# ACMMM2021-Anonymous/video-graph-ssl

Hardware: AMD Instinct MI355X
Metric: pretrain_clips_per_sec (higher is better)
Workload: dtype bf16x6 (fp32 tensors; conv products as 6 bf16 MFMAs on hi/mid/lo splits = fp32-grade, fp32 accumulate; everything else fp32)

## Files before the change

include/gca_hip.h:

```cpp
#ifndef GCA_HIP_H
#define GCA_HIP_H

#include <stdint.h>

#ifdef __cplusplus
extern "C" {
#endif

#define GCA_OK 0
#define GCA_EINVAL (-1)
#define GCA_ELAUNCH (-2)

int gca_version(void);

int gca_conv_halo_occupancy(int tm, int tn, int math, int64_t lds_bytes);

int gca_set_conv_math(int mode);
int gca_get_conv_math(void);

typedef struct {
  int32_t N, C, D, H, W;
  int32_t K;
  int32_t kd, kh, kw;
  int32_t sd, sh, sw;
  int32_t pd, ph, pw;
  int32_t OD, OH, OW;
  int64_t x_batch_stride;
  int32_t tune_fwd_bm, tune_fwd_splits;
  int32_t tune_dgrad_bm, tune_dgrad_splits;
  int32_t tune_wgrad_splits, tune_wgrad_tile;
  int32_t tune_fwd_tail, tune_dgrad_tail;
  int32_t tune_fwd_math, tune_dgrad_math, tune_wgrad_math;
  int32_t tune_fwd_box, tune_dgrad_box;
  int32_t act_f16;
} gca_conv_geom;

int64_t gca_conv_pack_elems(const gca_conv_geom* g, int which);
int gca_conv_pack(const gca_conv_geom* g, int which, const float* w, float* packed, void* stream);

#define GCA_PACK_JOB_BYTES 128
int64_t gca_conv_pack_jobs_host(const gca_conv_geom* g, int which, const float* w, float* packed, void* jobs_out);
int64_t gca_conv_pack_jobs_finalize_host(void* jobs, int64_t njobs);
int gca_conv_pack_batched(const void* jobs_dev, int64_t njobs, int64_t total_blocks, void* stream);

int64_t gca_conv_table_rows(const gca_conv_geom* g, int which);
int gca_conv_table_build_host(const gca_conv_geom* g, int which, int32_t* table_host );

int64_t gca_conv_fwd_stat_parts(const gca_conv_geom* g);
int gca_conv_kernel_cfg(const gca_conv_geom* g, int which, int32_t* out4);
int64_t gca_conv_pack_layout(const gca_conv_geom* g, int which);
int64_t gca_conv_fwd_ws_bytes(const gca_conv_geom* g);
int gca_conv_fwd(const gca_conv_geom* g, const void* x, const float* wpack, const int32_t* table,
                 const float* bias, void* y, float* stat_sum, float* stat_sq, void* ws, void* stream);

int64_t gca_conv_dgrad_ws_bytes(const gca_conv_geom* g);
int gca_conv_dgrad(const gca_conv_geom* g, const void* dy, const float* wpack, const int32_t* table,
                   void* dx, int accumulate, void* ws, void* stream);

int64_t gca_conv_wgrad_ws_bytes(const gca_conv_geom* g);
int gca_conv_wgrad(const gca_conv_geom* g, const void* x, const void* dy, const int32_t* table,
                   float* dw, int accumulate, void* ws, void* stream);
typedef struct {
  const float* slabs;
  float* dw;
  int64_t n;
  int32_t splits, accumulate;
  int32_t first_block, nblocks;
} gca_reduce_job;
int gca_conv_wgrad_partial(const gca_conv_geom* g, const void* x, const float* in_scale, const float* in_shift, const void* dy,
                           const int32_t* table, void* slabs, int32_t* out_splits, void* stream);

int gca_conv_xf_ok(const gca_conv_geom* g);
int gca_conv_fwd_xf(const gca_conv_geom* g, const void* x, const float* in_scale, const float* in_shift, const float* wpack,
                    const int32_t* table, const float* bias, void* y, float* stat_sum, float* stat_sq, void* ws, void* stream);
int gca_conv_wgrad_xf(const gca_conv_geom* g, const void* x, const float* in_scale, const float* in_shift, const void* dy,
                      const int32_t* table, float* dw, int accumulate, void* ws, void* stream);
int gca_conv_dzf_ok(const gca_conv_geom* g);
int gca_conv_wgrad_dzf(const gca_conv_geom* g, const void* x, const void* dz, const void* y, const float* consts, int relu,
                       const int32_t* table, float* dw, int accumulate, void* ws, void* stream);
int gca_conv_wgrad_dzf_partial(const gca_conv_geom* g, const void* x, const void* dz, const void* y, const float* consts, int relu,
                               const int32_t* table, void* slabs, int32_t* out_splits, void* stream);
int64_t gca_reduce_jobs_finalize_host(gca_reduce_job* jobs, int64_t njobs);
int gca_splitk_reduce_batched(const gca_reduce_job* jobs_dev, int64_t njobs, int64_t total_blocks, void* stream);
int gca_conv_wgrad_cfg(const gca_conv_geom* g, int32_t* out4);

int gca_bias_grad(const float* dy, int64_t N, int64_t K, int64_t SP, float* db, int accumulate, void* stream);

int gca_bn_stats(const void* x, int64_t N, int64_t C, int64_t SP, float* stat_sum, float* stat_sq,
                 int64_t* parts_out, int act_f16, void* stream);
int64_t gca_bn_stats_parts(int64_t N, int64_t C, int64_t SP);
int gca_bn_finalize(const float* stat_sum, const float* stat_sq, int64_t P, int64_t C, double count,
                    const float* gamma, const float* beta, float eps, float momentum,
                    float* running_mean, float* running_var, int64_t* num_batches_tracked,
                    float* save_mean, float* save_invstd, float* scale, float* shift, void* stream);
int gca_conv_fwd_slabs(const gca_conv_geom* g, const void* x, const float* wpack, const int32_t* table, void* ws,
                       int32_t* out_splits, void* stream);
int gca_bn_train_fwd_slabs(const float* slabs, int64_t splits, double count, const float* gamma, const float* beta, float eps,
                           float momentum, float* running_mean, float* running_var, int64_t* num_batches_tracked,
                           float* save_mean, float* save_invstd, float* scale, float* shift, float* y, const float* residual,
                           int relu, int64_t N, int64_t C, int64_t SP, float* z, int64_t z_batch_stride, void* stream);
int gca_bn_train_fwd(const float* stat_sum, const float* stat_sq, int64_t P, int64_t C, double count,
                     const float* gamma, const float* beta, float eps, float momentum,
                     float* running_mean, float* running_var, int64_t* num_batches_tracked,
                     float* save_mean, float* save_invstd, float* scale, float* shift,
                     const void* x, const void* residual, int relu, int64_t N, int64_t SP, void* z,
                     int64_t z_batch_stride, int act_f16, void* stream);
int gca_bn_fold_eval(const float* gamma, const float* beta, const float* running_mean,
                     const float* running_var, float eps, int64_t C, float* scale, float* shift, void* stream);
int gca_bn_apply(const void* x, const float* scale, const float* shift, const void* residual,
                 int relu, int64_t N, int64_t C, int64_t SP, void* z, int64_t z_batch_stride, int act_f16, void* stream);
// ... 131 lines not shown
```

video-graph-ssl_amd/_hip.py:

```python
import ctypes as C
import os

import torch

_HERE = os.path.dirname(os.path.abspath(__file__))
LIB_PATH = os.environ.get('GCA_LIB_PATH') or os.path.join(_HERE, 'libgca_hip.so')


class HipLibraryMissing(RuntimeError):
    pass


if not os.path.exists(LIB_PATH):
    raise HipLibraryMissing(
        'libgca_hip.so is not built (%s). Run ./build_hip.sh or __graft_entry__.build(); there is no '
        'CPU fallback for the product path.' % LIB_PATH)
lib = C.CDLL(LIB_PATH)

c_i32, c_i64, c_f32, c_f64, c_vp = C.c_int32, C.c_int64, C.c_float, C.c_double, C.c_void_p


class ConvGeom(C.Structure):
    _fields_ = [(n, c_i32) for n in ('N', 'C', 'D', 'H', 'W', 'K', 'kd', 'kh', 'kw', 'sd', 'sh', 'sw',
                                     'pd', 'ph', 'pw', 'OD', 'OH', 'OW')] + [('x_batch_stride', c_i64)] + \
               [(n, c_i32) for n in ('tune_fwd_bm', 'tune_fwd_splits', 'tune_dgrad_bm', 'tune_dgrad_splits',
                                     'tune_wgrad_splits', 'tune_wgrad_tile', 'tune_fwd_tail', 'tune_dgrad_tail',
                                     'tune_fwd_math', 'tune_dgrad_math', 'tune_wgrad_math', 'tune_fwd_box',
                                     'tune_dgrad_box', 'act_f16')]


class PoolGeom(C.Structure):
    _fields_ = [(n, c_i32) for n in ('N', 'C', 'D', 'H', 'W', 'kd', 'kh', 'kw', 'sd', 'sh', 'sw',
                                     'pd', 'ph', 'pw', 'OD', 'OH', 'OW')]


_GP, _PP = C.POINTER(ConvGeom), C.POINTER(PoolGeom)
SIGNATURES = {
    'gca_version': (c_i32, []),
    'gca_conv_halo_occupancy': (c_i32, [c_i32, c_i32, c_i32, c_i64]),
    'gca_set_conv_math': (c_i32, [c_i32]),
    'gca_get_conv_math': (c_i32, []),
    'gca_conv_pack_elems': (c_i64, [_GP, c_i32]),
    'gca_conv_pack': (c_i32, [_GP, c_i32, c_vp, c_vp, c_vp]),
    'gca_conv_table_rows': (c_i64, [_GP, c_i32]),
    'gca_conv_table_build_host': (c_i32, [_GP, c_i32, c_vp]),
    'gca_conv_fwd_stat_parts': (c_i64, [_GP]),
    'gca_conv_kernel_cfg': (c_i32, [_GP, c_i32, c_vp]),
    'gca_conv_pack_layout': (c_i64, [_GP, c_i32]),
    'gca_conv_fwd_ws_bytes': (c_i64, [_GP]),
    'gca_conv_fwd': (c_i32, [_GP, c_vp, c_vp, c_vp, c_vp, c_vp, c_vp, c_vp, c_vp, c_vp]),
    'gca_conv_dgrad_ws_bytes': (c_i64, [_GP]),
    'gca_conv_dgrad': (c_i32, [_GP, c_vp, c_vp, c_vp, c_vp, c_i32, c_vp, c_vp]),
    'gca_conv_wgrad_cfg': (c_i32, [_GP, c_vp]),
    'gca_conv_wgrad_ws_bytes': (c_i64, [_GP]),
    'gca_conv_wgrad': (c_i32, [_GP, c_vp, c_vp, c_vp, c_vp, c_i32, c_vp, c_vp]),
    'gca_bias_grad': (c_i32, [c_vp, c_i64, c_i64, c_i64, c_vp, c_i32, c_vp]),
    'gca_bn_stats': (c_i32, [c_vp, c_i64, c_i64, c_i64, c_vp, c_vp, c_vp, c_i32, c_vp]),
    'gca_bn_stats_parts': (c_i64, [c_i64, c_i64, c_i64]),
    'gca_bn_finalize': (c_i32, [c_vp, c_vp, c_i64, c_i64, c_f64, c_vp, c_vp, c_f32, c_f32, c_vp, c_vp, c_vp,
                                c_vp, c_vp, c_vp, c_vp, c_vp]),
    'gca_bn_train_fwd': (c_i32, [c_vp, c_vp, c_i64, c_i64, c_f64, c_vp, c_vp, c_f32, c_f32, c_vp, c_vp, c_vp,
                                 c_vp, c_vp, c_vp, c_vp, c_vp, c_vp, c_i32, c_i64, c_i64, c_vp, c_i64, c_i32, c_vp]),
    'gca_bn_fold_eval': (c_i32, [c_vp, c_vp, c_vp, c_vp, c_f32, c_i64, c_vp, c_vp, c_vp]),
    'gca_bn_apply': (c_i32, [c_vp, c_vp, c_vp, c_vp, c_i32, c_i64, c_i64, c_i64, c_vp, c_i64, c_i32, c_vp]),
    'gca_bn_bwd_ws_bytes': (c_i64, [c_i64, c_i64, c_i64]),
    'gca_bn_bwd': (c_i32, [c_vp, c_vp, c_vp, c_vp, c_vp, c_vp, c_i32, c_i64, c_i64, c_i64, c_vp, c_vp, c_vp,
                           c_vp, c_i32, c_i64, c_vp, c_vp, c_vp, c_i32, c_vp]),
    'gca_maxpool3d_fwd': (c_i32, [_PP, c_vp, c_vp, c_vp, c_vp, c_vp, c_i32, c_vp]),
    'gca_maxpool3d_bwd': (c_i32, [_PP, c_vp, c_vp, c_vp, c_i32, c_i32, c_vp]),
    'gca_avgpool3d_fwd': (c_i32, [_PP, c_vp, c_vp, c_vp]),
    'gca_avgpool3d_bwd': (c_i32, [_PP, c_vp, c_vp, c_i32, c_vp]),
    'gca_wavgpool_fwd': (c_i32, [c_vp, c_vp, c_f32, c_i64, c_i64, c_i64, c_vp, c_i32, c_vp]),
    'gca_wavgpool_bwd': (c_i32, [c_vp, c_vp, c_f32, c_i64, c_i64, c_i64, c_vp, c_i32, c_vp]),
    'gca_relu_fwd': (c_i32, [c_vp, c_i64, c_vp, c_vp]),
    'gca_relu_bwd': (c_i32, [c_vp, c_vp, c_i64, c_vp, c_vp]),
    'gca_l2norm_fwd': (c_i32, [c_vp, c_i64, c_i64, c_f32, c_vp, c_vp, c_vp]),
    'gca_l2norm_bwd': (c_i32, [c_vp, c_vp, c_vp, c_i64, c_i64, c_vp, c_vp]),
    'gca_negcos_fwd_bwd': (c_i32, [c_vp, c_vp, c_i64, c_i64, c_f32, c_vp, c_i32, c_vp, c_vp]),
    'gca_infonce_ws_bytes': (c_i64, [c_i64, c_i64]),
    'gca_moco_logits_fwd': (c_i32, [c_vp, c_vp, c_vp, c_i64, c_i64, c_i64, c_f32, c_vp, c_vp, c_vp, c_vp, c_vp, c_vp, c_vp]),
    'gca_nce_softmax_loss_fwd': (c_i32, [c_vp, c_i64, c_i64, c_vp, c_vp, c_vp, c_vp]),
    'gca_nce_softmax_loss_bwd': (c_i32, [c_vp, c_vp, c_i64, c_i64, c_vp, c_f32, c_vp, c_vp]),
    'gca_moco_logits_bwd': (c_i32, [c_vp, c_vp, c_vp, c_vp, c_f32, c_vp, c_vp, c_i64, c_i64, c_i64, c_f32,
                                    c_i64, c_vp, c_i64, c_vp, c_vp, c_vp, c_vp]),
    'gca_queue_enqueue': (c_i32, [c_vp, c_i64, c_i64, c_vp, c_i64, c_i64, c_vp, c_vp, c_vp]),
    'gca_queue_advance': (c_i32, [c_vp, c_i64, c_i64, c_vp]),
    'gca_graph_gram_ws_bytes': (c_i64, [c_i64, c_i64, c_i64, c_i64]),
    'gca_graph_adj_fwd': (c_i32, [c_vp, c_vp, c_i64, c_i64, c_i64, c_i64, c_i32, c_f32, c_f32, c_vp, c_vp,
                                  c_vp, c_vp, c_vp, c_vp]),
    'gca_graph_adj_bwd': (c_i32, [c_vp, c_vp, c_vp, c_vp, c_vp, c_vp, c_i64, c_i64, c_i64, c_i64, c_i32, c_f32,
                                  c_f32, c_vp, c_vp, c_vp]),
    'gca_graph_gcn_fwd': (c_i32, [c_vp, c_vp, c_i64, c_i64, c_i64, c_i64, c_vp, c_vp]),
    'gca_graph_gcn_bwd_ws_bytes': (c_i64, [c_i64, c_i64, c_i64, c_i64]),
    'gca_graph_gcn_bwd': (c_i32, [c_vp, c_vp, c_vp, c_i64, c_i64, c_i64, c_i64, c_vp, c_vp, c_vp, c_vp]),
    'gca_ema_update': (c_i32, [c_vp, c_vp, c_i64, c_f32, c_vp]),
    'gca_sgd_step': (c_i32, [c_vp, c_vp, c_vp, c_i64, c_vp, c_vp, c_f32, c_f32, c_i32, c_i32, c_vp, c_vp]),
    'gca_lars_job_chunks': (c_i32, []),
    'gca_lars_step': (c_i32, [c_vp, c_vp, c_vp, c_i64, c_vp, c_vp, c_vp, c_i64, c_vp, c_vp, c_i64, c_vp, c_vp, c_vp, c_vp, c_f32,
                              c_i32, c_f64, c_f64, c_vp, c_vp]),
    'gca_adam_step': (c_i32, [c_vp, c_vp, c_vp, c_vp, c_i64, c_vp, c_vp, c_f64, c_f64, c_f64, c_i32, c_vp, c_vp, c_vp]),
    'gca_adam_advance': (c_i32, [c_vp, c_vp, c_vp]),
    'gca_grad_clip_ws_bytes': (c_i64, []),
    'gca_grad_clip_coef': (c_i32, [c_vp, c_i64, c_f32, c_vp, c_vp, c_vp]),
    'gca_conv_wgrad_partial': (c_i32, [_GP, c_vp, c_vp, c_vp, c_vp, c_vp, c_vp, c_vp, c_vp]),
    'gca_conv_xf_ok': (c_i32, [_GP]),
# ... 87 lines not shown
```

video-graph-ssl_amd/csrc/conv3d.hip:

```cpp
#include <cstring>
#include <type_traits>
#include "conv_halo.h"

#include <cstdlib>
#include <vector>

using namespace gca_conv;

namespace {


constexpr int LDK = BK + 4;
constexpr int lds_pitch(int math) { return math == 2 ? 28 : (math == 3 ? 12 : LDK); }
constexpr int lds_bufs(int tm, bool vec, int math) { return (math >= 1 || vec || tm >= 4) ? 1 : 2; }
constexpr int cmax(int a, int b) { return a > b ? a : b; }

template <int TM, int BN, int FAST, bool VEC, int MATH, bool H = false>
__device__ __forceinline__ void igemm_tile(
    const void* __restrict__ src, const float* __restrict__ apack, const int2* __restrict__ table,
    const float* __restrict__ bias, void* __restrict__ dst, float* __restrict__ psum,
    float* __restrict__ psq, float* __restrict__ slab, const IgemmParams p, int bid,
    float* __restrict__ As_, float* __restrict__ Bs_, int* __restrict__ taptab) {
  constexpr unsigned ES = H ? 2u : 4u;
  constexpr int BM = 32 * TM, TN = BN / 128;
// ... 537 lines not shown
      for (int r = 0; r < 16; ++r) {
        float s = 0.f, q = 0.f;
#pragma unroll
        for (int j = 0; j < TN; ++j) { const float v = acc[i][j][r]; s += v; q += v * v; }
        s = half_wave_sum_hi(s);
        q = half_wave_sum_hi(q);
        const int ro = i * 32 + (r & 3) + 8 * (r >> 2) + 4 * lh;
        if (ll == 31) { red[(wn * BM + ro) * 2] = s; red[(wn * BM + ro) * 2 + 1] = q; }
      }
    }
    __syncthreads();
    if (tid < BM && mbase + tid < p.DK) {
      const float s = red[tid * 2] + red[(BM + tid) * 2] + red[(2 * BM + tid) * 2] + red[(3 * BM + tid) * 2];
      const float q = red[tid * 2 + 1] + red[(BM + tid) * 2 + 1] + red[(2 * BM + tid) * 2 + 1] + red[(3 * BM + tid) * 2 + 1];
      const long long m = mbase + tid;
      psum[m * p.P + tileN] = s;
      psq[m * p.P + tileN] = q;
    }
  }
}

template <int TM, int BN, int FAST, bool VEC, int MATH, bool H = false>
__global__ __launch_bounds__(256) void conv_igemm_kernel(
    const void* __restrict__ src, const float* __restrict__ apack, const int2* __restrict__ table,
    const float* __restrict__ bias, void* __restrict__ dst, float* __restrict__ psum,
    float* __restrict__ psq, float* __restrict__ slab, IgemmParams p) {
  __shared__ __attribute__((aligned(16))) float As_[lds_bufs(TM, VEC, MATH) * 32 * TM * lds_pitch(MATH)];
  __shared__ __attribute__((aligned(16))) float Bs_[lds_bufs(TM, VEC, MATH) * BN * lds_pitch(MATH)];
  __shared__ int taptab[64];
  igemm_tile<TM, BN, FAST, VEC, MATH, H>(src, apack, table, bias, dst, psum, psq, slab, p, gca_xcd_remap(blockIdx.x, gridDim.x), As_, Bs_,
                                   taptab);
}

template <int TMA, int TMB, int FAST, int MATH>
__global__ __launch_bounds__(256) void conv_igemm_2phase_kernel(
    const void* __restrict__ src, const float* __restrict__ apack, const int2* __restrict__ table,
    const float* __restrict__ bias, void* __restrict__ dst, float* __restrict__ psum,
    float* __restrict__ psq, IgemmParams p, int nA, int tilesM_B, int tilesN_B) {
  static_assert(TMB < TMA, "the tail uses the shorter tile");
  __shared__ __attribute__((aligned(16))) float As_[cmax(lds_bufs(TMA, false, MATH) * TMA, lds_bufs(TMB, false, MATH) * TMB) * 32 * lds_pitch(MATH)];
  __shared__ __attribute__((aligned(16))) float Bs_[cmax(lds_bufs(TMA, false, MATH), lds_bufs(TMB, false, MATH)) * 128 * lds_pitch(MATH)];
  __shared__ int taptab[64];
  if ((int)blockIdx.x < nA) {
    igemm_tile<TMA, 128, FAST, false, MATH>(src, apack, table, bias, dst, psum, psq, nullptr, p, gca_xcd_remap(blockIdx.x, nA), As_, Bs_, taptab);
  } else {
    IgemmParams pb = p;
    pb.tileN_off = p.tileN_off + p.tilesN;
    pb.tilesM = tilesM_B; pb.tilesN = tilesN_B;
    igemm_tile<TMB, 128, FAST, false, MATH>(src, apack, table, bias, dst, psum, psq, nullptr, pb,
                                      gca_xcd_remap((int)blockIdx.x - nA, (int)gridDim.x - nA), As_, Bs_, taptab);
  }
}

constexpr int FINISH_CHUNK = 1024;
template <typename T>
__global__ __launch_bounds__(256) void conv_splitk_finish_kernel(
    const float* __restrict__ slab, int splits, const float* __restrict__ bias, T* __restrict__ dst,
    float* __restrict__ psum, float* __restrict__ psq, IgemmParams p) {
  __shared__ double sh[4];
  const int m = blockIdx.x, part = blockIdx.y, P = gridDim.y;
  const float b = bias ? bias[m] : 0.f;
  const long long lo = (long long)part * FINISH_CHUNK;
  long long hi = lo + FINISH_CHUNK; if (hi > p.Ntot) hi = p.Ntot;
  const int QSP = p.QD * p.QH * p.QW, QHW = p.QH * p.QW, DHW = p.DH * p.DW;
  const long long DSP = (long long)p.DD * DHW;
  double s = 0.0, q = 0.0;
  for (long long n = lo + threadIdx.x; n < hi; n += 256) {
    float v = 0.f;
    const float* sp0 = slab + (long long)m * p.Ntot + n;
    const long long sstride = (long long)p.DK * p.Ntot;
    int k = 0;
    for (; k + 4 <= splits; k += 4) {
      const float l0 = sp0[(long long)k * sstride], l1 = sp0[(long long)(k + 1) * sstride];
      const float l2 = sp0[(long long)(k + 2) * sstride], l3 = sp0[(long long)(k + 3) * sstride];
      v += l0; v += l1; v += l2; v += l3;
    }
    for (; k < splits; ++k) v += sp0[(long long)k * sstride];
    s += (double)v; q += (double)v * (double)v;
    v += b;
    const int img = (int)(n / QSP);
    const int sp = (int)(n - (long long)img * QSP);
    const int qd = sp / QHW, rr = sp - qd * QHW;
    const int qh = rr / p.QW, qw = rr - qh * p.QW;
    const long long dsp = (long long)(qd * p.dm_d + p.do_d) * DHW + (qh * p.dm_h + p.do_h) * p.DW + (qw * p.dm_w + p.do_w);
    T* d = dst + ((long long)img * p.DK + m) * DSP + dsp;
    if (p.accumulate) v += (float)*d;
    *d = (T)v;
  }
  if (psum) {
    s = gca_block_sum256_d(s, sh);
    q = gca_block_sum256_d(q, sh);
    if (threadIdx.x == 0) { psum[(long long)m * P + part] = (float)s; psq[(long long)m * P + part] = (float)q; }
  }
}

__device__ __forceinline__ void pack_elements(const float* __restrict__ w, float* __restrict__ packed,
                                              const PackParams& p, long long first, long long step, long long end) {
  for (long long i = first; i < end; i += step) {
    const int m = (int)(i / p.Kpad), k = (int)(i - (long long)m * p.Kpad);
    float v = 0.f;
    if (m < p.M && k < p.Kred) {
      const int ch = k / p.ntaps, tl = k - ch * p.ntaps;
      const int a = tl / (p.nb * p.nc), r = tl - a * (p.nb * p.nc), b = r / p.nc, c = r - b * p.nc;
      const int tap = ((p.k0d + p.sd * a) * p.KH + (p.k0h + p.sh * b)) * p.KW + (p.k0w + p.sw * c);
      v = w[(long long)ch * p.s_ch + tap + (long long)m * p.s_m];
    }
    packed[i] = v;
  }
}
__global__ void conv_pack_kernel(const float* __restrict__ w, float* __restrict__ packed, PackParams p) {
  if (p.fmt >= 1)
    pack_halo_elements(w, reinterpret_cast<unsigned char*>(packed), p, (long long)blockIdx.x * blockDim.x + threadIdx.x,
                       (long long)gridDim.x * blockDim.x, pack_items(p));
  else
    pack_elements(w, packed, p, (long long)blockIdx.x * blockDim.x + threadIdx.x, (long long)gridDim.x * blockDim.x,
                  pack_items(p));
}

constexpr int PACK_CHUNK = 2048;
struct PackJob {
  PackParams p;
  const float* w;
  float* packed;
  int first_block, nblocks;
};
static_assert(sizeof(PackJob) <= GCA_PACK_JOB_BYTES, "gca_hip.h: GCA_PACK_JOB_BYTES too small");
__global__ __launch_bounds__(256) void conv_pack_batched_kernel(const unsigned char* __restrict__ jobs, int njobs) {
  const int bid = blockIdx.x;
  int lo = 0, hi = njobs - 1;
  while (lo < hi) {
    const int mid = (lo + hi + 1) >> 1;
    if (reinterpret_cast<const PackJob*>(jobs + (size_t)mid * GCA_PACK_JOB_BYTES)->first_block <= bid) lo = mid;
    else hi = mid - 1;
  }
  const PackJob* j = reinterpret_cast<const PackJob*>(jobs + (size_t)lo * GCA_PACK_JOB_BYTES);
  const PackParams p = j->p;
  const long long base = (long long)(bid - j->first_block) * PACK_CHUNK;
  long long end = base + PACK_CHUNK;
  const long long total = pack_items(p);
  if (end > total) end = total;
  if (p.fmt >= 1) pack_halo_elements(j->w, reinterpret_cast<unsigned char*>(j->packed), p, base + threadIdx.x, 256, end);
  else pack_elements(j->w, j->packed, p, base + threadIdx.x, 256, end);
}

__global__ void zero_fill_kernel(unsigned* __restrict__ p, long long n32, int tail16) {
  for (long long i = (long long)blockIdx.x * blockDim.x + threadIdx.x; i < n32; i += (long long)gridDim.x * blockDim.x) p[i] = 0u;
// ... 387 lines not shown
  return pw_launch(pw, src, reinterpret_cast<const unsigned char*>(apack), bias, dst, psum, psq, st);
}

int run_class_stem(const gca_conv_geom* g, const IgemmCfg& cf, const float* src, const float* apack, const float* bias, float* dst,
                   float* psum, float* psq, const IgemmParams& p, hipStream_t st) {
  StemParams sp;
  if (!stem_geometry(g, p, cf.math, sp) || sp.bd != cf.bd || sp.bh != cf.bh || sp.bw != cf.bw) return GCA_EINVAL;
  sp.g.splits = 1; sp.g.kt_per_split = sp.nsteps;
  sp.g.tilesM = cdiv(p.DK, 32 * sp.wm);
  const long long tn = (long long)g->N * sp.nbd * sp.nbh * sp.nbw;
  if (tn > 0x7fffffffLL) return GCA_EINVAL;
  sp.g.tilesN = (int)tn; sp.g.tileN_off = 0;
  sp.g.P = (int)tn;
  return stem_launch(cf.math, sp, src, reinterpret_cast<const unsigned char*>(apack), bias, dst, psum, psq, st);
}

struct ConvLaunch {
  std::vector<ClassInfo> cls;
  std::vector<IgemmParams> p;
  std::vector<IgemmCfg> cf;
};

ConvLaunch resolve_launch(const gca_conv_geom* g, int which) {
  ConvLaunch L;
  build_classes(g, which, L.cls);
  const size_t n = L.cls.size();
  L.p.assign(n, IgemmParams{});
  L.cf.assign(n, IgemmCfg{});
  for (size_t i = 0; i < n; ++i) {
    if (L.cls[i].ntaps == 0) continue;
    class_params(g, which, L.cls[i], L.p[i]);
    L.cf[i] = cfg_for(g, which, L.cls[i], L.p[i], n);
  }
  return L;
}

int run_resolved_class(const gca_conv_geom* g, int which, const ConvLaunch& L, size_t i, const float* src, const float* apack,
                       const int2* table, const float* bias, float* dst, float* psum, float* psq, float* slab, int accumulate,
                       hipStream_t st, bool leave_slabs = false, const float* in_scale = nullptr, const float* in_shift = nullptr) {
  const ClassInfo& c = L.cls[i];
  const IgemmCfg& cf = L.cf[i];
  IgemmParams p = L.p[i];
  p.accumulate = accumulate ? 1 : 0;
  switch (cf.kernel) {
    case ConvKernel::Pointwise: return run_class_pw(g, which, src, apack, bias, dst, psum, psq, p, st);
    case ConvKernel::Stem: return run_class_stem(g, cf, src, apack, bias, dst, psum, psq, p, st);
    case ConvKernel::Halo:
      return run_class_halo(g, c, cf, src, apack, table, bias, dst, psum, psq, slab, p, st, leave_slabs, in_scale, in_shift);
    case ConvKernel::Gather: break;
  }
  return run_class(cf, fast_of(c.ntaps), src, apack, table, bias, dst, psum, psq, slab, p, st, leave_slabs);
}

int64_t ws_bytes_for(const gca_conv_geom* g, int which) {
  const ConvLaunch L = resolve_launch(g, which);
  int64_t need = 0;
  for (size_t i = 0; i < L.cls.size(); ++i)
    if (L.cf[i].splits > 1) need = std::max<int64_t>(need, (int64_t)L.cf[i].splits * L.p[i].DK * L.p[i].Ntot * (int64_t)sizeof(float));
  return need;
}

int g_conv_math = -1;

}

namespace gca_conv {
int conv_math() {
  if (g_conv_math < 0) {
    const char* e = getenv("GCA_CONV_MATH");
    g_conv_math = !e ? 2 : (!strcmp(e, "bf16x3") || !strcmp(e, "1")) ? 1 : (!strcmp(e, "f32") || !strcmp(e, "0")) ? 0 : 2;
  }
  return g_conv_math;
}
}

extern "C" {

int gca_version(void) { return 15; }

int gca_set_conv_math(int mode) {
  if (mode < 0 || mode > 2) return GCA_EINVAL;
  g_conv_math = mode;
  return GCA_OK;
}
int gca_get_conv_math(void) { return conv_math(); }

int64_t gca_conv_pack_elems(const gca_conv_geom* g, int which) {
  if (!geom_ok(g) || (which != 0 && which != 1)) return GCA_EINVAL;
  int64_t n = 0;
  for (const ClassInfo& c : resolve_launch(g, which).cls) n += pack_reserve(c);
  return n > 0 ? n : 64;
}

static void pack_params_of(const gca_conv_geom* g, int which, const ClassInfo& c, const IgemmCfg& cf, PackParams& p) {
  const int T = taps(g);
  p.fmt = (int)cf.kernel; p.math = cf.math; p.SC = c.srcC;
  p.nsteps = cf.kernel == ConvKernel::Stem ? cf.kt_per_split : cdiv(c.srcC, 16) * c.ntaps;
  const bool pwfmt = p.fmt == 3;
  p.Kred = (int)c.Kred; p.M = c.M; p.Kpad = pwfmt ? (int)gca_round_up(c.srcC, 32) : (int)c.Kpad; p.Mrows = pack_rows(c.M);
  p.ntaps = p.fmt == 2 ? g->kd * g->kh : c.ntaps; p.nb = c.nb; p.nc = c.nc;
  p.k0d = c.k0[0]; p.k0h = c.k0[1]; p.k0w = c.k0[2]; p.sd = c.ks[0]; p.sh = c.ks[1]; p.sw = c.ks[2];
  p.KH = g->kh; p.KW = g->kw; p.T = T;
  if (which == 0) { p.s_ch = T; p.s_m = (long long)g->C * T; }
  else { p.s_ch = (long long)g->C * T; p.s_m = T; }
}

int64_t gca_conv_pack_jobs_host(const gca_conv_geom* g, int which, const float* w, float* packed, void* jobs_out) {
  if (!geom_ok(g) || (which != 0 && which != 1)) return GCA_EINVAL;
  const ConvLaunch L = resolve_launch(g, which);
  int64_t n = 0;
  for (size_t i = 0; i < L.cls.size(); ++i) {
// ... 147 lines not shown
  if (!geom_ok(g)) return GCA_EINVAL;
  const ConvLaunch L = resolve_launch(g, 0);
  const IgemmCfg& cf = L.cf[0];
  if (cf.kernel == ConvKernel::Pointwise) return (int64_t)g->N * cdiv((int)((long long)g->OD * g->OH * g->OW), 128);
  return stat_parts(cf, L.p[0].Ntot, cf.kernel != ConvKernel::Gather ? halo_tiles_n(g, L.cls[0], cf) : 0);
}

int64_t gca_conv_fwd_ws_bytes(const gca_conv_geom* g) { return geom_ok(g) ? ws_bytes_for(g, 0) : GCA_EINVAL; }
int64_t gca_conv_dgrad_ws_bytes(const gca_conv_geom* g) { return geom_ok(g) ? ws_bytes_for(g, 1) : GCA_EINVAL; }

int gca_conv_fwd(const gca_conv_geom* g, const void* x_, const float* wpack, const int32_t* table,
                 const float* bias, void* y_, float* stat_sum, float* stat_sq, void* ws, void* stream) {
  const float* x = reinterpret_cast<const float*>(x_);
  float* y = reinterpret_cast<float*>(y_);
  if (!geom_ok(g) || !x || !wpack || !table || !y) return GCA_EINVAL;
  if ((stat_sum == nullptr) != (stat_sq == nullptr)) return GCA_EINVAL;
  return run_resolved_class(g, 0, resolve_launch(g, 0), 0, x, wpack, reinterpret_cast<const int2*>(table), bias, y, stat_sum,
                            stat_sq, reinterpret_cast<float*>(ws), 0, (hipStream_t)stream);
}

int gca_conv_fwd_slabs(const gca_conv_geom* g, const void* x, const float* wpack, const int32_t* table, void* ws,
                       int32_t* out_splits, void* stream) {
  if (!out_splits || !ws || !x || !wpack || !table || !geom_ok(g) || g->act_f16) return GCA_EINVAL;
  const ConvLaunch L = resolve_launch(g, 0);
  const IgemmCfg& cf = L.cf[0];
  if ((cf.kernel != ConvKernel::Gather && cf.kernel != ConvKernel::Halo) || cf.splits < 2) return GCA_EINVAL;
  float* slab = reinterpret_cast<float*>(ws);
  const int rc = run_resolved_class(g, 0, L, 0, reinterpret_cast<const float*>(x), wpack, reinterpret_cast<const int2*>(table),
                                    nullptr, slab, nullptr, nullptr, slab, 0, (hipStream_t)stream, true);
  if (rc) return rc;
  *out_splits = cf.splits;
  return GCA_OK;
}

int gca_conv_xf_ok(const gca_conv_geom* g) {
  if (!geom_ok(g) || g->act_f16) return 0;
  const IgemmCfg cf = resolve_launch(g, 0).cf[0];
  if (cf.kernel != ConvKernel::Halo || cf.math == 3) return 0;
  return resolve_wgrad(g).xf ? 1 : 0;
}

int gca_conv_fwd_xf(const gca_conv_geom* g, const void* x_, const float* in_scale, const float* in_shift, const float* wpack,
                    const int32_t* table, const float* bias, void* y_, float* stat_sum, float* stat_sq, void* ws, void* stream) {
  const float* x = reinterpret_cast<const float*>(x_);
  float* y = reinterpret_cast<float*>(y_);
  if (!geom_ok(g) || g->act_f16 || !x || !in_scale || !in_shift || !wpack || !table || !y) return GCA_EINVAL;
  if ((stat_sum == nullptr) != (stat_sq == nullptr)) return GCA_EINVAL;
  const ConvLaunch L = resolve_launch(g, 0);
  if (L.cf[0].kernel != ConvKernel::Halo) return GCA_EINVAL;
  return run_resolved_class(g, 0, L, 0, x, wpack, reinterpret_cast<const int2*>(table), bias, y, stat_sum, stat_sq,
                            reinterpret_cast<float*>(ws), 0, (hipStream_t)stream, false, in_scale, in_shift);
}

int gca_conv_dgrad(const gca_conv_geom* g, const void* dy_, const float* wpack, const int32_t* table,
                   void* dx_, int accumulate, void* ws, void* stream) {
  const float* dy = reinterpret_cast<const float*>(dy_);
  float* dx = reinterpret_cast<float*>(dx_);
  if (!geom_ok(g) || !dy || !wpack || !table || !dx) return GCA_EINVAL;
  if (g->x_batch_stride != 0 && g->x_batch_stride != (long long)g->C * g->D * g->H * g->W) return GCA_EINVAL;
  hipStream_t st = (hipStream_t)stream;
  const ConvLaunch L = resolve_launch(g, 1);
  bool any_empty = false;
  for (const ClassInfo& c : L.cls) any_empty |= c.ntaps == 0;
  if (any_empty && !accumulate) {
    const long long n = (long long)g->N * g->C * g->D * g->H * g->W;
    const long long n32 = g->act_f16 ? n / 2 : n;
    long long blocks = gca_ceil_div(n32 + 1, 1024);
    if (blocks > 4096) blocks = 4096;
    hipLaunchKernelGGL(zero_fill_kernel, dim3((unsigned)blocks), dim3(256), 0, st, reinterpret_cast<unsigned*>(dx), n32,
                       g->act_f16 ? (int)(n & 1) : 0);
  }
  const int2* tab = reinterpret_cast<const int2*>(table);
  for (size_t i = 0; i < L.cls.size(); ++i) {
    const ClassInfo& c = L.cls[i];
    if (c.ntaps == 0) continue;
    const int rc = run_resolved_class(g, 1, L, i, dy, wpack + c.pack_off, tab + c.table_off, nullptr, dx, nullptr, nullptr,
                                      reinterpret_cast<float*>(ws), accumulate, st);
    if (rc) return rc;
  }
  return GCA_OK;
}

}
```

video-graph-ssl_amd/csrc/conv_igemm_host.h:

```cpp
#pragma once
#include <algorithm>
#include <vector>
#include "conv_common.h"

namespace gca_conv {

struct IgemmParams {
  int SC, SD, SH, SW;
  int DK;
  int QD, QH, QW;
  int DD, DH, DW;
  int dm_d, dm_h, dm_w;
  int do_d, do_h, do_w;
  int m_d, m_h, m_w;
  int o_d, o_h, o_w;
  int ntaps;
  int Kpad, Mpad;
  int tilesM, tilesN;
  int tileN_off;
  int splits, kt_per_split;
  int P;
  int chk;
  int accumulate;
  long long Ntot;
  long long src_nstride;
  unsigned src_bytes;
  unsigned dst_bytes;
  unsigned slab_bytes;
};

struct ClassInfo {
  int na, nb, nc, ntaps;
  int k0[3], ks[3];
  int dl0[3], dls[3];
  int q[3];
  int dm[3], dof[3];
  int m[3], o[3];
  int srcC, M;
  long long Kred, Kpad;
  long long table_off;
  long long pack_off;
  bool vec;
};

inline int cdiv(int a, int b) { return (a + b - 1) / b; }
inline int fast_of(int ntaps) { return ntaps <= 31 ? 1 : (ntaps <= FAST_MAX_TAPS ? 2 : 0); }
inline int pack_rows(int M) { return (int)gca_round_up(M, 32) + 128; }

inline long long pack_reserve(const ClassInfo& c) {
  const long long rows = pack_rows(c.M);
  const long long flat = c.Kpad * rows;
  const long long halo = c.srcC >= 8 && c.ntaps <= 64 ? (long long)cdiv(c.srcC, 16) * c.ntaps * rows * 24 : 0;
  const long long stem = c.srcC <= 4 && c.nc <= 8 && c.m[2] == 2 ? (long long)cdiv(c.srcC * c.na * c.nb, 2) * rows * 24 : 0;
  const long long m = halo > stem ? halo : stem;
  return m > flat ? m : flat;
}

inline void build_classes(const gca_conv_geom* g, int which, std::vector<ClassInfo>& out) {
  const int kdim[3] = {g->kd, g->kh, g->kw}, sdim[3] = {g->sd, g->sh, g->sw}, pdim[3] = {g->pd, g->ph, g->pw};
  const int in[3] = {g->D, g->H, g->W}, od[3] = {g->OD, g->OH, g->OW};
  long long toff = 0, poff = 0;
  auto finish = [&](ClassInfo& c) {
    c.ntaps = c.na * c.nb * c.nc;
    c.Kred = (long long)c.srcC * c.ntaps;
    c.Kpad = gca_round_up(c.Kred, BK);
    c.table_off = toff; c.pack_off = poff;
    toff += c.Kpad + 32;
    poff += pack_reserve(c);
    const int SH = which == 0 ? in[1] : od[1], SW = which == 0 ? in[2] : od[2];
    c.vec = c.nb == 1 && c.nc == 1 && c.m[1] == 1 && c.m[2] == 1 && c.o[1] + c.dl0[1] == 0 && c.o[2] + c.dl0[2] == 0 &&
            c.dm[1] == 1 && c.dm[2] == 1 && c.dof[1] == 0 && c.dof[2] == 0 && c.q[1] == SH && c.q[2] == SW &&
            (SH * SW) % 4 == 0 && c.ntaps <= 31 &&
            (which == 1 || g->x_batch_stride % 4 == 0);
    out.push_back(c);
  };
  if (which == 0) {
    ClassInfo c{};
    c.na = g->kd; c.nb = g->kh; c.nc = g->kw;
    for (int d = 0; d < 3; ++d) {
      c.k0[d] = 0; c.ks[d] = 1; c.dl0[d] = 0; c.dls[d] = 1;
      c.q[d] = od[d]; c.dm[d] = 1; c.dof[d] = 0; c.m[d] = sdim[d]; c.o[d] = -pdim[d];
    }
// ... 84 lines not shown
```

video-graph-ssl_amd/engine/ops.py:

```python
import ctypes as C
import functools
import os

import torch

from .. import _hip as H
from .._hip import aptr, is_half, ptr, stream
from . import tune
from .tune import TUNE_HALO, TUNE_PW, TUNE_STEM, TUNE_VEC

F32 = torch.float32
F16 = torch.float16


def _t3(v):
    return (v, v, v) if isinstance(v, int) else tuple(int(a) for a in v)


class _Workspace:

    def __init__(self):
        self.buf = {}
        self.captured = set()
        self.retired = []
# ... 66 lines not shown

if _TUNE_PATH:
    import atexit
    if os.path.exists(_TUNE_PATH):
        load_tune_cache(_TUNE_PATH)
    atexit.register(lambda: _TUNE_DIRTY[0] and os.environ.get('RANK', '0') == '0' and save_tune_cache(_TUNE_PATH))


def _time_ms(fn, reps=3):
    fn()
    a, b = torch.cuda.Event(enable_timing=True), torch.cuda.Event(enable_timing=True)
    a.record()
    for _ in range(reps):
        fn()
    b.record()
    b.synchronize()
    return a.elapsed_time(b) / reps


_KERNELS = (('halo', TUNE_HALO, 14), ('stem', TUNE_STEM, 16), ('pw', TUNE_PW, 17))


def _tune_kernel(code):
    return next((name for name, flag, _ in _KERNELS if code & flag), 'gather')


class ConvPlan:

    def __init__(self, N, Cin, D, Hh, W, K, k, s, p, device, x_batch_stride=0, act_f16=False):
        kd, kh, kw = _t3(k)
        sd, sh, sw = _t3(s)
        pd, ph, pw = _t3(p)
        OD, OH, OW = (D + 2 * pd - kd) // sd + 1, (Hh + 2 * ph - kh) // sh + 1, (W + 2 * pw - kw) // sw + 1
        self.g = H.ConvGeom(N, Cin, D, Hh, W, K, kd, kh, kw, sd, sh, sw, pd, ph, pw, OD, OH, OW, x_batch_stride)
        self.g.act_f16 = int(bool(act_f16))
        self.act_dtype = F16 if act_f16 else F32
        self.gp = C.byref(self.g)
        self.in_shape = (N, Cin, D, Hh, W)
        self.out_shape = (N, K, OD, OH, OW)
        self.device = device
        self.taps = kd * kh * kw
        self._tables = {}
        self.tuned = [not AUTOTUNE] * 3
        if H.lib.gca_conv_fwd_stat_parts(self.gp) < 0:
            raise ValueError('unsupported conv geometry %r' % ((N, Cin, D, Hh, W, K, k, s, p),))
        self.pack_elems = [H.lib.gca_conv_pack_elems(self.gp, 0), H.lib.gca_conv_pack_elems(self.gp, 1)]
        self.refresh()

    def refresh(self):
        self.parts = H.lib.gca_conv_fwd_stat_parts(self.gp)
        self.wgrad_ws = H.lib.gca_conv_wgrad_ws_bytes(self.gp)
        self.fwd_ws = H.lib.gca_conv_fwd_ws_bytes(self.gp)
        self.dgrad_ws = H.lib.gca_conv_dgrad_ws_bytes(self.gp) if self.g.x_batch_stride == 0 else 0

    def table(self, which):
        t = self._tables.get(which)
        if t is None:
            rows = H.lib.gca_conv_table_rows(self.gp, which)
            host = torch.empty(rows * 2, dtype=torch.int32)
            H.call('gca_conv_table_build_host', self.gp, which, host.data_ptr())
            t = host.to(self.device)
            self._tables[which] = t
        return t

    def cfg(self, which):
        out = (C.c_int32 * 4)()
        if which == 2:
            H.call('gca_conv_wgrad_cfg', self.gp, out)
        else:
            H.call('gca_conv_kernel_cfg', self.gp, which, out)
        return tuple(out)

    WGRAD_KERNELS = {11: 'temporal32', 12: 'temporal64', 13: 'spatial', 14: 'stem'}
    WGRAD_SHAPES = tune.WGRAD_SHAPES

    def kernel(self, which):
        kc = self.cfg(which)[3]
        if which == 2:
            return self.WGRAD_KERNELS.get(kc & 255, 'gather')
        return next((name for name, _, bit in _KERNELS if kc >> bit & 1), 'gather')

    def math(self, which):
        return self.cfg(which)[3] >> 12 & 3

    def pack_layout(self, which):
        return 0 if which == 2 else H.lib.gca_conv_pack_layout(self.gp, which)

    def tune_key(self, which):
        g = self.g
        geom = (g.N, g.C, g.D, g.H, g.W, g.K, g.kd, g.kh, g.kw, g.sd, g.sh, g.sw, g.pd, g.ph, g.pw, g.x_batch_stride)
        return 'v%d%s:%d:%s' % (H.lib.gca_version(), 'h' if g.act_f16 else ('', 'b', 'c')[H.lib.gca_get_conv_math()], which,
                                ','.join(str(int(v)) for v in geom))

    def set_code(self, which, code):
        for field, v in zip(code._fields, code):
            setattr(self.g, 'tune_%s_%s' % (tune.PASSES[which], field), v)
        self.refresh()

    def tune(self, which, run, repack=None):
        if self.tuned[which] or torch.cuda.is_current_stream_capturing():
            return

        def measure():
            try:
                return _time_ms(run)
            except RuntimeError:
# ... 63 lines not shown

def conv_pack(plan, which, w, out=None):
    n = plan.pack_elems[which]
    if out is None or out.numel() != n:
        out = torch.zeros(n, dtype=F32, device=w.device)
    H.call('gca_conv_pack', plan.gp, which, ptr(w), ptr(out), stream())
    return out


def _act(plan, t):
    if t.dtype is not plan.act_dtype:
        raise TypeError('conv plan built for %s activations, got %s' % (plan.act_dtype, t.dtype))
    return aptr(t)


def _conv_fwd_launch(plan, x, wpack, bias, y, ss, sq):
    ws = WS.get(plan.fwd_ws, x.device) if plan.fwd_ws else None
    H.call('gca_conv_fwd', plan.gp, _act(plan, x), ptr(wpack), ptr(plan.table(0)), ptr(bias), _act(plan, y), ptr(ss), ptr(sq),
           ptr(ws), stream())


def _repacker(plan, which, w_raw, wpack):
    if w_raw is None:
        return None
    return lambda: H.call('gca_conv_pack', plan.gp, which, ptr(w_raw), ptr(wpack), stream())


def _stat_pair(plan, device):
    return tuple(torch.empty((plan.g.K, plan.parts), dtype=F32, device=device) for _ in range(2))


def conv_fwd(plan, x, wpack, bias=None, stats=False, w_raw=None):
    y = torch.empty(plan.out_shape, dtype=plan.act_dtype, device=x.device)
    if not plan.tuned[0]:
        plan.tune(0, lambda: _conv_fwd_launch(plan, x, wpack, bias, y, None, None), _repacker(plan, 0, w_raw, wpack))
    ss, sq = _stat_pair(plan, x.device) if stats else (None, None)
    _conv_fwd_launch(plan, x, wpack, bias, y, ss, sq)
    return (y, (ss, sq)) if stats else y


def conv_xf_ok(plan):
    return plan.tuned[0] and plan.tuned[2] and plan.g.x_batch_stride == 0 and bool(H.lib.gca_conv_xf_ok(plan.gp))


def conv_fwd_xf(plan, y_in, scale, shift, wpack, stats=False):
    y = torch.empty(plan.out_shape, dtype=F32, device=y_in.device)
    ss, sq = _stat_pair(plan, y_in.device) if stats else (None, None)
    ws = WS.get(plan.fwd_ws, y_in.device) if plan.fwd_ws else None
    H.call('gca_conv_fwd_xf', plan.gp, ptr(y_in), ptr(scale), ptr(shift), ptr(wpack), ptr(plan.table(0)), None, ptr(y), ptr(ss),
           ptr(sq), ptr(ws), stream())
    return (y, (ss, sq)) if stats else y


def _conv_dgrad_launch(plan, dy, wpack_t, dx, accumulate):
    ws = WS.get(plan.dgrad_ws, dy.device) if plan.dgrad_ws else None
    H.call('gca_conv_dgrad', plan.gp, _act(plan, dy), ptr(wpack_t), ptr(plan.table(1)), _act(plan, dx), int(accumulate), ptr(ws),
           stream())


def conv_dgrad(plan, dy, wpack_t, dx=None, accumulate=False, w_raw=None):
    if dx is None:
        dx = torch.empty(plan.in_shape, dtype=plan.act_dtype, device=dy.device)
        accumulate = False
    if not plan.tuned[1]:
        scratch = torch.empty(plan.in_shape, dtype=plan.act_dtype, device=dy.device)
        plan.tune(1, lambda: _conv_dgrad_launch(plan, dy, wpack_t, scratch, False), _repacker(plan, 1, w_raw, wpack_t))
    _conv_dgrad_launch(plan, dy, wpack_t, dx, accumulate)
    return dx


def _conv_wgrad_launch(plan, x, dy, dw, accumulate):
    ws = WS.get(plan.wgrad_ws, x.device)
    H.call('gca_conv_wgrad', plan.gp, _act(plan, x), _act(plan, dy), ptr(plan.table(2)), ptr(dw), int(accumulate), ptr(ws), stream())


class DeferredReduce(object):

    def __init__(self):
        self.slabs = {}
        self.tables = {}
        self.pending = []
        self.launches = 0

    def slab_for(self, dw, plan):
        key = (dw.data_ptr(), id(plan))
        b = self.slabs.get(key)
        if b is None or b.numel() < plan.wgrad_ws:
            if torch.cuda.is_current_stream_capturing():
                raise RuntimeError('weight-gradient slab would be allocated during graph capture; run one eager step first')
            b = self.slabs[key] = torch.empty(max(int(plan.wgrad_ws), 16), dtype=torch.uint8, device=dw.device)
        return b

    def add(self, plan, x, dy, dw, accumulate, xf=None, dzf=None):
        if any(j[1].data_ptr() == dw.data_ptr() for j in self.pending):
            self.flush()
        slab = self.slab_for(dw, plan)
        splits = C.c_int32(0)
        if dzf is not None:
            H.call('gca_conv_wgrad_dzf_partial', plan.gp, _act(plan, x), _act(plan, dy), _act(plan, dzf[0]), ptr(dzf[1]),
                   int(dzf[2]), ptr(plan.table(2)), slab.data_ptr(), C.addressof(splits), stream())
        else:
            H.call('gca_conv_wgrad_partial', plan.gp, _act(plan, x), ptr(xf[0]) if xf else None, ptr(xf[1]) if xf else None,
                   _act(plan, dy), ptr(plan.table(2)), slab.data_ptr(), C.addressof(splits), stream())
        self.pending.append((slab, dw, dw.numel(), int(splits.value), int(bool(accumulate))))

    def flush(self):
        if not self.pending:
            return
        jobs, self.pending = self.pending, []
        sig = tuple((j[0].data_ptr(), j[1].data_ptr(), j[2], j[3], j[4]) for j in jobs)
# ... 607 lines not shown
```

Before: 1656.

## Merge per-class strided dgrad launches into one multi-class kernel launch

Strided-conv dgrad used to issue a separate implicit-GEMM launch (plus a split-K finish launch) for each tap class. Now, when all classes share a tile config, one grouped kernel covers them, picking each workgroup's class from a prefix table passed as a kernel argument, and one finish kernel covers all split-K parts. This cuts launch count and lets classes fill the GPU together. In exchange the workspace grows to the sum of all class slabs instead of the max, and each block does a small class lookup.

```diff
diff --git a/include/gca_hip.h b/include/gca_hip.h
--- a/include/gca_hip.h
+++ b/include/gca_hip.h
@@ -56,6 +56,13 @@
 int64_t gca_conv_dgrad_ws_bytes(const gca_conv_geom* g);
 int gca_conv_dgrad(const gca_conv_geom* g, const void* dy, const float* wpack, const int32_t* table,
                    void* dx, int accumulate, void* ws, void* stream);
+#define GCA_CLASS_BLOCK_BYTES 2048
+int gca_conv_dgrad_merged(const gca_conv_geom* g, int64_t ws_bytes);
+int64_t gca_conv_dgrad_ws_bytes_merged(const gca_conv_geom* g);
+int gca_conv_dgrad_ws(const gca_conv_geom* g, const void* dy, const float* wpack, const int32_t* table,
+                      void* dx, int accumulate, void* ws, int64_t ws_bytes, void* stream);
+int gca_set_dgrad_merge(int on);
+int64_t gca_conv_class_block_bytes(void);
 
 int64_t gca_conv_wgrad_ws_bytes(const gca_conv_geom* g);
 int gca_conv_wgrad(const gca_conv_geom* g, const void* x, const void* dy, const int32_t* table,
diff --git a/video-graph-ssl_amd/_hip.py b/video-graph-ssl_amd/_hip.py
--- a/video-graph-ssl_amd/_hip.py
+++ b/video-graph-ssl_amd/_hip.py
@@ -51,6 +51,11 @@
     'gca_conv_fwd': (c_i32, [_GP, c_vp, c_vp, c_vp, c_vp, c_vp, c_vp, c_vp, c_vp, c_vp]),
     'gca_conv_dgrad_ws_bytes': (c_i64, [_GP]),
     'gca_conv_dgrad': (c_i32, [_GP, c_vp, c_vp, c_vp, c_vp, c_i32, c_vp, c_vp]),
+    'gca_conv_dgrad_ws_bytes_merged': (c_i64, [_GP]),
+    'gca_conv_dgrad_ws': (c_i32, [_GP, c_vp, c_vp, c_vp, c_vp, c_i32, c_vp, c_i64, c_vp]),
+    'gca_conv_dgrad_merged': (c_i32, [_GP, c_i64]),
+    'gca_set_dgrad_merge': (c_i32, [c_i32]),
+    'gca_conv_class_block_bytes': (c_i64, []),
     'gca_conv_wgrad_cfg': (c_i32, [_GP, c_vp]),
     'gca_conv_wgrad_ws_bytes': (c_i64, [_GP]),
     'gca_conv_wgrad': (c_i32, [_GP, c_vp, c_vp, c_vp, c_vp, c_i32, c_vp, c_vp]),
diff --git a/video-graph-ssl_amd/csrc/conv3d.hip b/video-graph-ssl_amd/csrc/conv3d.hip
--- a/video-graph-ssl_amd/csrc/conv3d.hip
+++ b/video-graph-ssl_amd/csrc/conv3d.hip
@@ -613,13 +613,32 @@
   }
 }
 
+__device__ __forceinline__ int class_of(const int* __restrict__ first, int id) {
+  int ci = 0;
+#pragma unroll
+  for (int i = 1; i < MAX_MERGED_CLASSES; ++i) ci += id >= first[i] ? 1 : 0;
+  return ci;
+}
+
+template <int TM, int BN, int FAST, bool VEC, int MATH, bool H = false>
+__global__ __launch_bounds__(256) void conv_igemm_classes_kernel(
+    const void* __restrict__ src, const float* __restrict__ apack, const int2* __restrict__ table, void* __restrict__ dst,
+    float* __restrict__ slab, const ClassBlock cb) {
+  __shared__ __attribute__((aligned(16))) float As_[lds_bufs(TM, VEC, MATH) * 32 * TM * lds_pitch(MATH)];
+  __shared__ __attribute__((aligned(16))) float Bs_[lds_bufs(TM, VEC, MATH) * BN * lds_pitch(MATH)];
+  __shared__ int taptab[64];
+  const int ci = class_of(cb.first_wg, (int)blockIdx.x);
+  const int first = cb.first_wg[ci], count = cb.first_wg[ci + 1] - first;
+  igemm_tile<TM, BN, FAST, VEC, MATH, H>(src, apack + cb.pack_off[ci], table + cb.table_off[ci], nullptr, dst, nullptr, nullptr,
+                                         slab + cb.slab_off[ci], cb.p[ci], gca_xcd_remap((int)blockIdx.x - first, count), As_, Bs_,
+                                         taptab);
+}
+
 constexpr int FINISH_CHUNK = 1024;
 template <typename T>
-__global__ __launch_bounds__(256) void conv_splitk_finish_kernel(
+__device__ __forceinline__ void splitk_finish_part(
     const float* __restrict__ slab, int splits, const float* __restrict__ bias, T* __restrict__ dst,
-    float* __restrict__ psum, float* __restrict__ psq, IgemmParams p) {
-  __shared__ double sh[4];
-  const int m = blockIdx.x, part = blockIdx.y, P = gridDim.y;
+    float* __restrict__ psum, float* __restrict__ psq, const IgemmParams& p, int m, int part, int P, double* sh) {
   const float b = bias ? bias[m] : 0.f;
   const long long lo = (long long)part * FINISH_CHUNK;
   long long hi = lo + FINISH_CHUNK; if (hi > p.Ntot) hi = p.Ntot;
@@ -653,6 +672,24 @@
     q = gca_block_sum256_d(q, sh);
     if (threadIdx.x == 0) { psum[(long long)m * P + part] = (float)s; psq[(long long)m * P + part] = (float)q; }
   }
+}
+
+template <typename T>
+__global__ __launch_bounds__(256) void conv_splitk_finish_kernel(
+    const float* __restrict__ slab, int splits, const float* __restrict__ bias, T* __restrict__ dst,
+    float* __restrict__ psum, float* __restrict__ psq, IgemmParams p) {
+  __shared__ double sh[4];
+  splitk_finish_part<T>(slab, splits, bias, dst, psum, psq, p, blockIdx.x, blockIdx.y, gridDim.y, sh);
+}
+
+template <typename T>
+__global__ __launch_bounds__(256) void conv_splitk_finish_classes_kernel(const float* __restrict__ slab, T* __restrict__ dst,
+                                                                         const ClassBlock cb) {
+  __shared__ double sh[4];
+  const int ci = class_of(cb.first_part, (int)blockIdx.y);
+  const int first = cb.first_part[ci];
+  splitk_finish_part<T>(slab + cb.slab_off[ci], cb.p[ci].splits, nullptr, dst, nullptr, nullptr, cb.p[ci], blockIdx.x,
+                        (int)blockIdx.y - first, cb.first_part[ci + 1] - first, sh);
 }
 
 __device__ __forceinline__ void pack_elements(const float* __restrict__ w, float* __restrict__ packed,
@@ -1146,11 +1183,126 @@
   return run_class(cf, fast_of(c.ntaps), src, apack, table, bias, dst, psum, psq, slab, p, st, leave_slabs);
 }
 
+inline int64_t class_slab_bytes(const IgemmCfg& cf, const IgemmParams& p) {
+  return cf.splits > 1 ? (int64_t)cf.splits * p.DK * p.Ntot * (int64_t)sizeof(float) : 0;
+}
+
+int g_dgrad_merge = -1;
+inline bool dgrad_merge_on() {
+  if (g_dgrad_merge < 0) {
+    const char* e = getenv("GCA_DGRAD_MERGE");
+    g_dgrad_merge = (e && !strcmp(e, "0")) ? 0 : (e && !strcmp(e, "2")) ? 2 : 1;
+  }
+  return g_dgrad_merge != 0;
+}
+
+template <int TM, int BN, int FAST, bool VEC>
+void launch_classes_one(int math, bool h, dim3 grid, hipStream_t st, const float* src, const float* apack, const int2* table,
+                        float* dst, float* slab, const ClassBlock& cb) {
+  if (h)
+    hipLaunchKernelGGL((conv_igemm_classes_kernel<TM, BN, FAST, VEC, 3, true>), grid, dim3(256), 0, st, src, apack, table, dst, slab, cb);
+  else if (math == 1)
+    hipLaunchKernelGGL((conv_igemm_classes_kernel<TM, BN, FAST, VEC, 1>), grid, dim3(256), 0, st, src, apack, table, dst, slab, cb);
+  else if (math == 2)
+    hipLaunchKernelGGL((conv_igemm_classes_kernel<TM, BN, FAST, VEC, 2>), grid, dim3(256), 0, st, src, apack, table, dst, slab, cb);
+  else
+    hipLaunchKernelGGL((conv_igemm_classes_kernel<TM, BN, FAST, VEC, 0>), grid, dim3(256), 0, st, src, apack, table, dst, slab, cb);
+}
+
+template <int TM>
+void launch_classes_tm(const IgemmCfg& c, int fast, dim3 grid, hipStream_t st, const float* src, const float* apack,
+                       const int2* table, float* dst, float* slab, const ClassBlock& cb) {
+  if (c.bn == 256) launch_classes_one<TM, 256, 1, true>(c.math, c.h, grid, st, src, apack, table, dst, slab, cb);
+  else if (fast == 1) launch_classes_one<TM, 128, 1, false>(c.math, c.h, grid, st, src, apack, table, dst, slab, cb);
+  else launch_classes_one<TM, 128, 2, false>(c.math, c.h, grid, st, src, apack, table, dst, slab, cb);
+}
+
+struct MergedLaunch {
+  ClassBlock cb;
+  IgemmCfg cf;
+  int fast;
+  long long wg, parts;
+  int64_t slab_bytes;
+};
+
+bool plan_merged(const ConvLaunch& L, int accumulate, MergedLaunch& m) {
+  m = MergedLaunch{};
+  ClassBlock& cb = m.cb;
+  int n = 0;
+  std::vector<size_t> order;
+  for (size_t i = 0; i < L.cls.size(); ++i)
+    if (L.cls[i].ntaps > 0) order.push_back(i);
+  if (g_dgrad_merge != 2)
+    std::stable_sort(order.begin(), order.end(), [&](size_t a, size_t b) { return L.cf[a].kt_per_split > L.cf[b].kt_per_split; });
+  for (const size_t i : order) {
+    const ClassInfo& c = L.cls[i];
+    const IgemmCfg& cf = L.cf[i];
+    const int fast = fast_of(c.ntaps);
+    if (n == MAX_MERGED_CLASSES || cf.kernel != ConvKernel::Gather || cf.tail_bm > 0 || fast == 0) return false;
+    if (n == 0) { m.cf = cf; m.fast = fast; }
+    else if (cf.bm != m.cf.bm || cf.bn != m.cf.bn || fast != m.fast || cf.math != m.cf.math || cf.h != m.cf.h) return false;
+    IgemmParams p = L.p[i];
+    p.accumulate = accumulate ? 1 : 0;
+    p.splits = cf.splits; p.kt_per_split = cf.kt_per_split;
+    p.P = stat_parts(cf, p.Ntot);
+    p.tilesM = (int)gca_ceil_div(p.DK, cf.bm);
+    p.tilesN = (int)gca_ceil_div(p.Ntot, cf.bn);
+    p.tileN_off = 0;
+    const long long nblk = (long long)p.tilesM * p.tilesN * cf.splits;
+    if (nblk <= 0 || (n > 0 && p.DK != cb.p[0].DK)) return false;
+    cb.p[n] = p;
+    cb.pack_off[n] = c.pack_off;
+    cb.table_off[n] = c.table_off;
+    cb.slab_off[n] = m.slab_bytes / (int64_t)sizeof(float);
+    cb.first_wg[n] = (int)m.wg;
+    cb.first_part[n] = (int)m.parts;
+    m.wg += nblk;
+    if (cf.splits > 1) m.parts += p.P;
+    m.slab_bytes += class_slab_bytes(cf, p);
+    if (m.wg > 0x7fffffffLL || m.parts > 65535) return false;
+    ++n;
+  }
+  if (n < 2) return false;
+  for (int i = n; i <= MAX_MERGED_CLASSES; ++i) { cb.first_wg[i] = 0x7fffffff; cb.first_part[i] = 0x7fffffff; }
+  cb.first_wg[n] = (int)m.wg;
+  cb.first_part[n] = (int)m.parts;
+  cb.n = n;
+  return true;
+}
+
+int run_classes_merged(const MergedLaunch& m, const float* dy, const float* wpack, const int2* tab, float* dx, float* ws,
+                       hipStream_t st) {
+  const ClassBlock& cb = m.cb;
+  const dim3 grid((unsigned)m.wg);
+  switch (m.cf.bm / 32) {
+    case 1: launch_classes_tm<1>(m.cf, m.fast, grid, st, dy, wpack, tab, dx, ws, cb); break;
+    case 2: launch_classes_tm<2>(m.cf, m.fast, grid, st, dy, wpack, tab, dx, ws, cb); break;
+    case 3: launch_classes_tm<3>(m.cf, m.fast, grid, st, dy, wpack, tab, dx, ws, cb); break;
+    case 4: launch_classes_tm<4>(m.cf, m.fast, grid, st, dy, wpack, tab, dx, ws, cb); break;
+    default: launch_classes_tm<5>(m.cf, m.fast, grid, st, dy, wpack, tab, dx, ws, cb); break;
+  }
+  const int rc = gca_launch_status();
+  if (rc || m.parts == 0) return rc;
+  const dim3 fgrid((unsigned)cb.p[0].DK, (unsigned)m.parts);
+  if (m.cf.h)
+    hipLaunchKernelGGL(conv_splitk_finish_classes_kernel<_Float16>, fgrid, dim3(256), 0, st, ws, reinterpret_cast<_Float16*>(dx), cb);
+  else
+    hipLaunchKernelGGL(conv_splitk_finish_classes_kernel<float>, fgrid, dim3(256), 0, st, ws, dx, cb);
+  return gca_launch_status();
+}
+
 int64_t ws_bytes_for(const gca_conv_geom* g, int which) {
   const ConvLaunch L = resolve_launch(g, which);
   int64_t need = 0;
   for (size_t i = 0; i < L.cls.size(); ++i)
     if (L.cf[i].splits > 1) need = std::max<int64_t>(need, (int64_t)L.cf[i].splits * L.p[i].DK * L.p[i].Ntot * (int64_t)sizeof(float));
+  return need;
+}
+
+int64_t ws_bytes_merged_for(const gca_conv_geom* g, int which) {
+  const ConvLaunch L = resolve_launch(g, which);
+  int64_t need = 0;
+  for (size_t i = 0; i < L.cls.size(); ++i) need += class_slab_bytes(L.cf[i], L.p[i]);
   return need;
 }
 
@@ -1404,8 +1556,23 @@
                             reinterpret_cast<float*>(ws), 0, (hipStream_t)stream, false, in_scale, in_shift);
 }
 
-int gca_conv_dgrad(const gca_conv_geom* g, const void* dy_, const float* wpack, const int32_t* table,
-                   void* dx_, int accumulate, void* ws, void* stream) {
+int64_t gca_conv_dgrad_ws_bytes_merged(const gca_conv_geom* g) { return geom_ok(g) ? ws_bytes_merged_for(g, 1) : GCA_EINVAL; }
+int64_t gca_conv_class_block_bytes(void) { return (int64_t)sizeof(ClassBlock); }
+int gca_conv_dgrad_merged(const gca_conv_geom* g, int64_t ws_bytes) {
+  if (!geom_ok(g)) return GCA_EINVAL;
+  const ConvLaunch L = resolve_launch(g, 1);
+  MergedLaunch m;
+  return L.cls.size() > 1 && dgrad_merge_on() && plan_merged(L, 0, m) && ws_bytes >= m.slab_bytes;
+}
+
+int gca_set_dgrad_merge(int on) {
+  const int was = dgrad_merge_on() ? 1 : 0;
+  g_dgrad_merge = on == 2 ? 2 : (on ? 1 : 0);
+  return was;
+}
+
+int gca_conv_dgrad_ws(const gca_conv_geom* g, const void* dy_, const float* wpack, const int32_t* table,
+                      void* dx_, int accumulate, void* ws, int64_t ws_bytes, void* stream) {
   const float* dy = reinterpret_cast<const float*>(dy_);
   float* dx = reinterpret_cast<float*>(dx_);
   if (!geom_ok(g) || !dy || !wpack || !table || !dx) return GCA_EINVAL;
@@ -1423,6 +1590,9 @@
                        g->act_f16 ? (int)(n & 1) : 0);
   }
   const int2* tab = reinterpret_cast<const int2*>(table);
+  MergedLaunch m;
+  if (L.cls.size() > 1 && dgrad_merge_on() && plan_merged(L, accumulate, m) && (m.slab_bytes == 0 || (ws && ws_bytes >= m.slab_bytes)))
+    return run_classes_merged(m, dy, wpack, tab, dx, reinterpret_cast<float*>(ws), st);
   for (size_t i = 0; i < L.cls.size(); ++i) {
     const ClassInfo& c = L.cls[i];
     if (c.ntaps == 0) continue;
@@ -1433,4 +1603,9 @@
   return GCA_OK;
 }
 
-}
+int gca_conv_dgrad(const gca_conv_geom* g, const void* dy, const float* wpack, const int32_t* table,
+                   void* dx, int accumulate, void* ws, void* stream) {
+  return gca_conv_dgrad_ws(g, dy, wpack, table, dx, accumulate, ws, geom_ok(g) && ws ? ws_bytes_for(g, 1) : 0, stream);
+}
+
+}
diff --git a/video-graph-ssl_amd/csrc/conv_igemm_host.h b/video-graph-ssl_amd/csrc/conv_igemm_host.h
--- a/video-graph-ssl_amd/csrc/conv_igemm_host.h
+++ b/video-graph-ssl_amd/csrc/conv_igemm_host.h
@@ -28,6 +28,18 @@
   unsigned dst_bytes;
   unsigned slab_bytes;
 };
+
+constexpr int MAX_MERGED_CLASSES = 8;
+struct ClassBlock {
+  IgemmParams p[MAX_MERGED_CLASSES];
+  long long pack_off[MAX_MERGED_CLASSES];
+  long long table_off[MAX_MERGED_CLASSES];
+  long long slab_off[MAX_MERGED_CLASSES];
+  int first_wg[MAX_MERGED_CLASSES + 1];
+  int first_part[MAX_MERGED_CLASSES + 1];
+  int n, pad_;
+};
+static_assert(sizeof(ClassBlock) <= GCA_CLASS_BLOCK_BYTES, "gca_hip.h: GCA_CLASS_BLOCK_BYTES too small");
 
 struct ClassInfo {
   int na, nb, nc, ntaps;
diff --git a/video-graph-ssl_amd/engine/ops.py b/video-graph-ssl_amd/engine/ops.py
--- a/video-graph-ssl_amd/engine/ops.py
+++ b/video-graph-ssl_amd/engine/ops.py
@@ -142,6 +142,7 @@
         self.wgrad_ws = H.lib.gca_conv_wgrad_ws_bytes(self.gp)
         self.fwd_ws = H.lib.gca_conv_fwd_ws_bytes(self.gp)
         self.dgrad_ws = H.lib.gca_conv_dgrad_ws_bytes(self.gp) if self.g.x_batch_stride == 0 else 0
+        self.dgrad_ws_merged = H.lib.gca_conv_dgrad_ws_bytes_merged(self.gp) if self.g.x_batch_stride == 0 else 0
 
     def table(self, which):
         t = self._tables.get(which)
@@ -311,10 +312,15 @@
     return (y, (ss, sq)) if stats else y
 
 
-def _conv_dgrad_launch(plan, dy, wpack_t, dx, accumulate):
-    ws = WS.get(plan.dgrad_ws, dy.device) if plan.dgrad_ws else None
-    H.call('gca_conv_dgrad', plan.gp, _act(plan, dy), ptr(wpack_t), ptr(plan.table(1)), _act(plan, dx), int(accumulate), ptr(ws),
-           stream())
+def set_dgrad_merge(on):
+    return bool(H.lib.gca_set_dgrad_merge(int(bool(on))))
+
+
+def _conv_dgrad_launch(plan, dy, wpack_t, dx, accumulate, ws_bytes=None):
+    need = max(plan.dgrad_ws, plan.dgrad_ws_merged) if ws_bytes is None else ws_bytes
+    ws = WS.get(need, dy.device) if need else None
+    H.call('gca_conv_dgrad_ws', plan.gp, _act(plan, dy), ptr(wpack_t), ptr(plan.table(1)), _act(plan, dx), int(accumulate), ptr(ws),
+           need, stream())
 
 
 def conv_dgrad(plan, dy, wpack_t, dx=None, accumulate=False, w_raw=None):
```

After: 1679, median of 6. 1.01x the previous value.
